# epitaque/RaytracingTest

Measured on AMD Instinct MI355X. Metric: Mrays/sec + achieved HBM GB/s, 1920x1080 primary rays, depth-10 SVO, higher is better.
Workload: dtype f32; 1 GPU; C3 depth-10 (1024^3) Custom1 SVO, 1920x1080 primary rays, flyover camera; svo_config=defaults, svo_nodes=1569748, svo_format=V2, stack_mode=hlsl, rays_per_gpu_step=2073600, parallelism=single

## Files before the change

raytracingtest_amd/csrc/svo_kernel.hip:

```cpp
#include "svo_traverse.h"
#include "svo_reflect.h"

#include <hipcub/hipcub.hpp>

namespace svo {
namespace {

__device__ __forceinline__ void mul4(const float *m, float v0, float v1, float v2, float v3, float out[3]) {
#pragma unroll
    for (int r = 0; r < 3; ++r) {
        float a = m[0 * 4 + r] * v0;
        a = a + m[1 * 4 + r] * v1;
        a = a + m[2 * 4 + r] * v2;
        a = a + m[3 * 4 + r] * v3;
        out[r] = a;
    }
}

__device__ __forceinline__ void normalize3(float v[3]) {
    float d = v[0] * v[0];
    d = d + v[1] * v[1];
    d = d + v[2] * v[2];
    float inv = 1.0f / sqrtf(d);
    v[0] = v[0] * inv;
// ... 684 lines not shown
        if (fin != 0) {
            if (SEGS && LM_ON(fin)) n_lane = (uint32_t)it;
            stopped |= stop;
            act &= ~fin;
            if (KG > 1) {
                recs |= fin & ~stop;
                act &= ~after_in_group<KG>(recs);
            }
        }
        asm volatile("s_cmp_lt_u32 %1, %2\n\ts_cselect_b64 %0, %3, 0" : "=s"(go) : "s"(it), "n"(MAX_ITERS), "s"(act) : "scc");
    } while (go != 0);
    if (LM_ON(act)) {
        r.flags |= 2u;
        if (SEGS) n_lane = (uint32_t)it;
    }
    stopped_lane = LM_ON(stopped);
    r.idx = sh ^ oct;
    r.trips = it;
}


__device__ __forceinline__ float beam_start(const LaunchParams &p, const FRay &f, int x, int gy) {
    if (!p.tile_start) return -__builtin_inff();
    const unsigned long long k = min(min(p.tile_start[(gy >> 3) * p.ts_tiles_x + (x >> 3)],
                                         p.tile_start[p.ts_super_off + (gy >> 6) * p.ts_super_x + (x >> 6)]),
                                     p.tile_start[p.ts_global_off]);
    const float d = (uint32_t)(k >> 32) == ~p.ts_gen ? __uint_as_float((uint32_t)k) : __builtin_inff();
    const float m = (2.0f * (fabsf(f.cx) + fabsf(f.cy) + fabsf(f.cz)) + fabsf(f.bx) + fabsf(f.by) + fabsf(f.bz)) *
                    0x1p-20f;
    const float s = d * (1.0f - 0x1p-16f) - m;
    return s == s ? s : -__builtin_inff();
}

template <int MODE, bool FA, bool COUNT = false, bool LOD = false>
__device__ __forceinline__ void trace_beam(const LaunchParams &p, FRay &f, uint2 *__restrict__ stk, float start) {
    uint32_t n_lane, armed_at;
    bool stopped;
    trace_seg<MODE, FA, false, COUNT, 0, LOD>(p, f, stk, start, __builtin_inff(), f.t_min >= start, n_lane, armed_at, stopped);
}

__device__ __forceinline__ int strip_col(int x, int m) {
    constexpr int K = STRIP_K;
    return K == 1 ? m * 8 + x : (m / K) * (8 * K) + x * K + (m % K);
}
__device__ __forceinline__ int strip_tile(int x, int e, int tiles_x, int tiles_y) {
    const int m = e / tiles_y, row = e - m * tiles_y;
    return row * tiles_x + strip_col(x, m);
}

template <int MODE, bool COUNT, bool FA, bool SH, bool LAT, bool LOD>
__device__ __forceinline__ void render_tile_body(const LaunchParams &p, int tiles_x) {
    static_assert(!(LOD && (SH || LAT)), "no LOD form of the fused shadow pass or the latency loop");
    extern __shared__ uint2 stk_base[];
    const int lane = threadIdx.x;
    const uint32_t t_entry = !COUNT && p.wave_log ? (uint32_t)__builtin_amdgcn_s_memrealtime() : 0u;
    const int n_tiles = (int)gridDim.x;
    const int t = p.tile_order ? (int)p.tile_order[blockIdx.x]
                : p.xcd_remap == 2 ? strip_tile((int)blockIdx.x % 8, (int)blockIdx.x / 8, tiles_x, n_tiles / tiles_x)
                                   : (int)blockIdx.x;
    const int bx = t % tiles_x, by = t / tiles_x;
    const int x = bx * 8 + (lane & 7);
    const int lr = by * 8 + (lane >> 3);
    if (x >= p.width || lr >= p.local_rows) return;
    if (p.tile_order && p.prio) {
        const uint32_t n = gridDim.x;
        const bool strips = p.xcd_remap == 2;
        const uint32_t b = strips ? blockIdx.x / 8 : blockIdx.x;
        const uint32_t *bound = strips ? p.tile_order + n + 4 + 4 * (blockIdx.x % 8) : p.tile_order + n;
        if (b < bound[0]) __builtin_amdgcn_s_setprio(3);
        else if (b < bound[1]) __builtin_amdgcn_s_setprio(2);
        else if (b < bound[2]) __builtin_amdgcn_s_setprio(1);
    }
    const int gy = global_row(p, lr);
    Ray r;
    {
        float org[3], dir[3];
        camera_ray(p.cam, p.width, p.height, x, gy, org, dir);
        setup_ray(org, dir, r);
    }
    uint2 *stk = stk_base + lane;
    uint32_t t0 = 0;
    if (!COUNT && p.wave_log) t0 = (uint32_t)__builtin_amdgcn_s_memrealtime();
    FRay f;
    to_fray(r, f);
    LeanDiag dg;
    if (LOD) {
        if (COUNT) {
            if (p.tile_start) trace_beam<MODE, false, true, true>(p, f, stk, fminf(beam_start(p, f, x, gy), p.lod_floor));
            else trace_lean<MODE, true, false, false, true, true>(p, f, stk);
        }
        else if (p.guard) trace_lean<MODE, true, false, false, false, true>(p, f, stk);
        else if (p.tile_start) trace_beam<MODE, FA, false, true>(p, f, stk, fminf(beam_start(p, f, x, gy), p.lod_floor));
        else trace_lean<MODE, false, false, FA, false, true>(p, f, stk);
    }
    else if (COUNT) {
        if (p.tile_start) trace_beam<MODE, false, true>(p, f, stk, beam_start(p, f, x, gy));
        else trace_lean<MODE, true, false, false, true>(p, f, stk);
    }
    else if (LAT) trace_lat<MODE>(p, f, stk);
    else if (!SH && p.wave_log) {
        if (p.guard) trace_lean<MODE, true, true>(p, f, stk, &dg);
        else trace_lean<MODE, false, true>(p, f, stk, &dg);
    }
    else if (p.guard) trace_lean<MODE, true>(p, f, stk);
    else if (p.tile_start) trace_beam<MODE, FA>(p, f, stk, beam_start(p, f, x, gy));
    else trace_lean<MODE, false, false, FA>(p, f, stk);
    from_fray(f, r);
    if (COUNT) {
        p.out.fetches[(size_t)lr * (size_t)p.width + (size_t)x] = r.fetches;
        return;
    }
    const float4 acc = accum_load(p, out_index(p, lr, gy, x));
    Record o;
    record(p, r, x, gy, o);
    int trips = f.trips;
    if (SH) {
        const bool hit = r.scale < S_MAX;
        const uint64_t hits = __ballot(hit);
        if (hits) {
            if (hit) {
                float so[3], sd[3];
                shadow_ray(p, x, gy, o.w[2], o.w[3], o.w[4], o.w[5], so, sd);
                Ray rs;
                setup_ray(so, sd, rs);
                FRay fs;
                to_fray(rs, fs);
                if (p.guard) trace_lean<MODE, true>(p, fs, stk);
                else trace_lean<MODE, false, false, FA>(p, fs, stk);
                from_fray(fs, rs);
                if (rs.scale < S_MAX) {
                    o.w[1] |= 8u << 16;
                    o.rgb[0] = o.rgb[1] = o.rgb[2] = 0.0f;
                }
                trips += fs.trips;
            }
            trips = __shfl(trips, __ffsll((long long)hits) - 1);
        }
    }
    if (p.out.hitmask) {
        const uint64_t hm = __ballot(r.scale < S_MAX);
        if (lane == 0) p.out.hitmask[t] = hm;
    }
    if (p.tile_cost && (!SH || lane == 0)) p.tile_cost[t] = (uint16_t)min(trips, 65535);
    if (p.wave_log && lane == 0) {
        uint32_t *w = p.wave_log + WAVE_LOG_WORDS * (size_t)blockIdx.x;
        w[8] = t_entry;
        w[10] = (uint32_t)__builtin_amdgcn_s_getreg((31 << 11) | 4);
        w[0] = t0;
        w[1] = (uint32_t)__builtin_amdgcn_s_memrealtime();
        w[2] = (uint32_t)t;
        w[3] = ((uint32_t)__builtin_amdgcn_s_getreg((31 << 11) | 20) & 0xFFu) | ((uint32_t)f.trips << 8);
        w[4] = (uint32_t)dg.loop_cycles;
        w[5] = (uint32_t)dg.fetch_cycles;
        w[6] = dg.fetch_trips;
        w[7] = dg.pop_trips;
    }
    store_outputs(p.out, out_index(p, lr, gy, x), o, acc);
    if (p.wave_log && lane == 0) p.wave_log[WAVE_LOG_WORDS * (size_t)blockIdx.x + 9] = (uint32_t)__builtin_amdgcn_s_memrealtime();
}

template <int MODE, bool COUNT, bool FA = false, bool SH = false, bool LAT = false>
#ifndef SVO_NUM_SGPR
#define SVO_NUM_SGPR 72
#endif
__global__ __launch_bounds__(TILE) __attribute__((amdgpu_num_sgpr(SVO_NUM_SGPR))) void render_tile_kernel(LaunchParams p, int tiles_x) {
    render_tile_body<MODE, COUNT, FA, SH, LAT, false>(p, tiles_x);
}

template <int MODE, bool COUNT, bool FA = false>
__global__ __launch_bounds__(TILE) __attribute__((amdgpu_num_sgpr(SVO_NUM_SGPR), amdgpu_waves_per_eu(8, 8)))
void render_tile_lod_kernel(LaunchParams p, int tiles_x) {
    render_tile_body<MODE, COUNT, FA, false, false, true>(p, tiles_x);
}

__device__ __forceinline__ int group_min(int v, int K) {
    v = min(v, __shfl_xor(v, 1));
    v = min(v, __shfl_xor(v, 2));
    if (K == 8) v = min(v, __shfl_xor(v, 4));
    return v;
}
__device__ __forceinline__ float group_get(float v, int K, int j) {
    return __shfl(v, (int)(threadIdx.x & ~(uint32_t)(K - 1)) + j);
}
__device__ __forceinline__ uint32_t group_get(uint32_t v, int K, int j) {
    return (uint32_t)__shfl((int)v, (int)(threadIdx.x & ~(uint32_t)(K - 1)) + j);
}

__device__ __forceinline__ void seg_rebalance(uint2 *slot, float t_entry, float t_start, float t_end, uint32_t c,
                                              int f, int K, float tot, float *hint8, bool store) {
    const int lane = (int)threadIdx.x, k = lane & (K - 1);
    slot[lane] = make_uint2(k <= f ? c : 0u, __float_as_uint(k == 0 ? t_entry : k > f ? t_end : t_start));
    __syncthreads();
    if (k != 0 || !store) return;
    if (!(tot > 0.0f)) {
        hint8[0] = __int_as_float(0x7FC00000);
        return;
    }
    const uint2 *g = slot + lane;
    int m = 0;
    float cum = 0.0f, cm = (float)g[0].x, t0 = t_entry, prev = 0.0f;
    float t1 = K > 1 ? __uint_as_float(g[1].y) : t_end;
// ... 80 lines not shown
    tot += (uint32_t)__shfl_xor((int)tot, 2);
    if (K == 8) tot += (uint32_t)__shfl_xor((int)tot, 4);
    seg_rebalance(stk_base, t_entry, t_start, t_end, c, fsel, K, (float)tot, hint8, inside && hint8);
    if (p.tile_cost) {
        uint32_t m = inside ? tot : 0u;
        for (int d = K; d < TILE; d <<= 1) m = max(m, (uint32_t)__shfl_xor((int)m, d));
        if (lane == 0) {
            p.part_cost[SEG_KMAX * (size_t)t + part] = (uint16_t)min(m, (uint32_t)(SEG_COST_FLAG - 1));
            if (part == 0) p.tile_cost[t] = (uint16_t)(SEG_COST_FLAG | K);
        }
    }
    if (p.out.hitmask) {
        uint32_t hit_w = (writer && inside && r.scale < S_MAX) ? 1u : 0u;
        hit_w |= (uint32_t)__shfl_xor((int)hit_w, 1);
        hit_w |= (uint32_t)__shfl_xor((int)hit_w, 2);
        if (K == 8) hit_w |= (uint32_t)__shfl_xor((int)hit_w, 4);
        const uint64_t hm = __ballot(k == 0 && hit_w != 0);
        uint32_t bits = 0;
#pragma unroll
        for (int j = 0; j < R; ++j) bits |= (uint32_t)((hm >> (K * j)) & 1ull) << j;
        if (lane == 0) {
            if (K == 4) reinterpret_cast<uint16_t *>(p.out.hitmask)[4 * (size_t)t + part] = (uint16_t)bits;
            else reinterpret_cast<uint8_t *>(p.out.hitmask)[8 * (size_t)t + part] = (uint8_t)bits;
        }
    }
    if (LOG) seg_log(p, 9, now_100mhz());
    if (!writer || !inside) return;
    const float4 acc = accum_load(p, out_index(p, lr, gy, x));
    Record o;
    record(p, r, x, gy, o);
    store_outputs(p.out, out_index(p, lr, gy, x), o, acc);
}

template <int MODE, bool FA, bool LAT, bool LOG>
#ifndef SVO_SEG_WAVES_PER_EU
#define SVO_SEG_WAVES_PER_EU 8
#endif
__global__ __launch_bounds__(TILE) __attribute__((amdgpu_num_sgpr(SVO_NUM_SGPR), amdgpu_waves_per_eu(SVO_SEG_WAVES_PER_EU, 8)))
void render_seg_kernel(LaunchParams p, int tiles_x) {
    extern __shared__ uint2 stk_base[];
    const int lane = threadIdx.x;
    const uint32_t t_in = LOG ? now_100mhz() : 0u;
    const uint32_t entry = p.tile_order[blockIdx.x];
    if (LOG) {
        seg_log(p, 8, t_in);
        seg_log(p, 2, entry);
    }
    if (entry == SEG_EMPTY) return;
    const int t = (int)(entry & 0x0FFFFFFFu);
    const int code = (int)(entry >> 28);
    if (p.prio) {
        const uint32_t *bound = p.tile_order + gridDim.x + 4 + 4 * (blockIdx.x % 8);
        const uint32_t b = blockIdx.x / 8;
        if (b < bound[0]) __builtin_amdgcn_s_setprio(3);
        else if (b < bound[1]) __builtin_amdgcn_s_setprio(2);
        else if (b < bound[2]) __builtin_amdgcn_s_setprio(1);
    }
    const int bx = t % tiles_x, by = t / tiles_x;
    uint2 *stk = stk_base + lane;
    if (code == 0) {
        const int x = bx * 8 + (lane & 7);
        const int lr = by * 8 + (lane >> 3);
        if (x >= p.width || lr >= p.local_rows) return;
        const int gy = global_row(p, lr);
        Ray r;
        {
            float org[3], dir[3];
            camera_ray(p.cam, p.width, p.height, x, gy, org, dir);
            setup_ray(org, dir, r);
        }
        FRay f;
        to_fray(r, f);
        if (LOG) seg_log(p, 0, now_100mhz());
        if (LAT) trace_lat<MODE>(p, f, stk);
        else if (p.tile_start) trace_beam<MODE, FA>(p, f, stk, beam_start(p, f, x, gy));
        else trace_lean<MODE, false, false, FA>(p, f, stk);
        if (LOG) {
            seg_log(p, 1, now_100mhz());
            seg_log(p, 3, ((uint32_t)__builtin_amdgcn_s_getreg((31 << 11) | 20) & 0xFFu) | ((uint32_t)f.trips << 8));
        }
        from_fray(f, r);
        const float4 acc = accum_load(p, out_index(p, lr, gy, x));
        Record o;
        record(p, r, x, gy, o);
        if (p.out.hitmask) {
            const uint64_t hm = __ballot(r.scale < S_MAX);
            if (lane == 0) p.out.hitmask[t] = hm;
        }
        if (p.tile_cost) p.tile_cost[t] = (uint16_t)min(f.trips, (int)(SEG_COST_FLAG - 1));
        store_outputs(p.out, out_index(p, lr, gy, x), o, acc);
        if (LOG) seg_log(p, 9, now_100mhz());
        return;
    }
    if (code <= 4) seg_part<MODE, FA, 4, LOG>(p, stk_base, t, code - 1, bx, by);
    else seg_part<MODE, FA, 8, LOG>(p, stk_base, t, code - 5, bx, by);
}

template <int MODE, bool FA, bool LOD>
__device__ __forceinline__ void render_samples_body(const LaunchParams &p, int tiles_x) {
    extern __shared__ uint2 stk_base[];
    const int lane = threadIdx.x & (TILE - 1);
    const int k = threadIdx.x / TILE;
    const int n_tiles = (int)gridDim.x;
    const int t = p.tile_order ? (int)p.tile_order[blockIdx.x]
                : p.xcd_remap == 2 ? strip_tile((int)blockIdx.x % 8, (int)blockIdx.x / 8, tiles_x, n_tiles / tiles_x)
                                   : (int)blockIdx.x;
    const int bx = t % tiles_x, by = t / tiles_x;
// ... 541 lines not shown
                rgb[0] = rgb[1] = rgb[2] = 0.0f;
            } else {
                float alb[3];
                decode_dxt(at.x, at.y, (int)(c.y & 0xFFu), alb);
                shade_hit(a.cam, n, alb, rgb);
            }
        }
    } else if (a.out.rgba || a.out.rgba8) {
        float org[3], dir[3];
        camera_ray(a.cam, a.width, a.height, x, y, org, dir);
        sky(dir[1], rgb);
    }
    if (a.out.hits) {
        uint2 *d = reinterpret_cast<uint2 *>(a.out.hits + dst);
        d[0] = make_uint2(c.x, c.y);
        d[1] = make_uint2(c.z, __float_as_uint(n[0]));
        d[2] = make_uint2(__float_as_uint(n[1]), __float_as_uint(n[2]));
    }
    if (a.out.rgba) a.out.rgba[dst] = make_float4(rgb[0], rgb[1], rgb[2], 1.0f);
    if (a.out.rgba8) a.out.rgba8[dst] = pack_rgba8(rgb[0], rgb[1], rgb[2]);
}

}

static size_t lds_pad() {
    static const size_t pad = [] {
        const char *v = std::getenv("SVO_LDS_PAD");
        return v ? (size_t)std::strtoul(v, nullptr, 10) : (size_t)0;
    }();
    return pad;
}

template <int MODE, bool COUNT>
static hipError_t launch_variant(const LaunchParams &p, hipStream_t stream) {
    const int bx = (p.width + 7) / 8, by = (p.local_rows + 7) / 8;
    const size_t lds = (size_t)p.slots * TILE * sizeof(uint2) + lds_pad();
    const dim3 grid((unsigned)(bx * by)), block(TILE);
    if (p.lod) {
        if (p.seg > 0 || p.lat || p.shadows) return hipErrorInvalidValue;
        const bool fa = p.fetch_all && !p.guard;
        if (COUNT)
            hipLaunchKernelGGL((render_tile_lod_kernel<MODE, true>), grid, block, lds, stream, p, bx);
        else if (p.samples > 0) {
            const size_t per = (size_t)std::max(p.slots, 2) * TILE * sizeof(uint2);
            const dim3 sblock((unsigned)(TILE * p.samples));
            if (fa) hipLaunchKernelGGL((render_samples_lod_kernel<MODE, true>), grid, sblock, per * p.samples, stream, p, bx);
            else hipLaunchKernelGGL((render_samples_lod_kernel<MODE, false>), grid, sblock, per * p.samples, stream, p, bx);
        } else if (fa)
            hipLaunchKernelGGL((render_tile_lod_kernel<MODE, false, true>), grid, block, lds, stream, p, bx);
        else
            hipLaunchKernelGGL((render_tile_lod_kernel<MODE, false, false>), grid, block, lds, stream, p, bx);
        return hipGetLastError();
    }
    if (!COUNT && p.samples > 0) {
        const size_t per = (size_t)std::max(p.slots, 2) * TILE * sizeof(uint2);
        const dim3 sblock((unsigned)(TILE * p.samples));
        if (p.fetch_all && !p.guard)
            hipLaunchKernelGGL((render_samples_kernel<MODE, true>), grid, sblock, per * p.samples, stream, p, bx);
        else
            hipLaunchKernelGGL((render_samples_kernel<MODE, false>), grid, sblock, per * p.samples, stream, p, bx);
        return hipGetLastError();
    }
    if (!COUNT && p.seg > 0) {
        const dim3 sgrid((unsigned)order_strips_grid(bx * by, p.seg, p.seg_kmax));
        if (p.lat && p.wave_log)
            hipLaunchKernelGGL((render_seg_kernel<MODE, true, true, true>), sgrid, block, 2 * lds, stream, p, bx);
        else if (p.lat)
            hipLaunchKernelGGL((render_seg_kernel<MODE, true, true, false>), sgrid, block, 2 * lds, stream, p, bx);
        else if (p.fetch_all && p.wave_log)
            hipLaunchKernelGGL((render_seg_kernel<MODE, true, false, true>), sgrid, block, lds, stream, p, bx);
        else if (p.fetch_all)
            hipLaunchKernelGGL((render_seg_kernel<MODE, true, false, false>), sgrid, block, lds, stream, p, bx);
        else if (p.wave_log)
            hipLaunchKernelGGL((render_seg_kernel<MODE, false, false, true>), sgrid, block, lds, stream, p, bx);
        else
            hipLaunchKernelGGL((render_seg_kernel<MODE, false, false, false>), sgrid, block, lds, stream, p, bx);
        return hipGetLastError();
    }
    if (COUNT)
        hipLaunchKernelGGL((render_tile_kernel<MODE, true>), grid, block, lds, stream, p, bx);
    else if (p.lat)
        hipLaunchKernelGGL((render_tile_kernel<MODE, false, false, false, true>), grid, block, 2 * lds, stream, p, bx);
    else if (p.shadows == 2) {
        if (p.fetch_all && !p.guard)
            hipLaunchKernelGGL((render_tile_kernel<MODE, false, true, true>), grid, block, lds, stream, p, bx);
        else
            hipLaunchKernelGGL((render_tile_kernel<MODE, false, false, true>), grid, block, lds, stream, p, bx);
    } else if (p.fetch_all && !p.guard)
        hipLaunchKernelGGL((render_tile_kernel<MODE, false, true>), grid, block, lds, stream, p, bx);
    else
        hipLaunchKernelGGL((render_tile_kernel<MODE, false>), grid, block, lds, stream, p, bx);
    return hipGetLastError();
}

template <int MODE>
static hipError_t launch_query_mode(const LaunchParams &p, const QueryArgs &q, hipStream_t stream) {
    const size_t lds = (size_t)p.slots * TILE * sizeof(uint2) + lds_pad();
    const dim3 grid((q.n + (uint32_t)TILE - 1u) / (uint32_t)TILE), block(TILE);
    if (p.lod) {
        if (p.guard)
            hipLaunchKernelGGL((query_rays_lod_kernel<MODE, true, false>), grid, block, lds, stream, p, q);
        else if (p.fetch_all)
            hipLaunchKernelGGL((query_rays_lod_kernel<MODE, false, true>), grid, block, lds, stream, p, q);
        else
            hipLaunchKernelGGL((query_rays_lod_kernel<MODE, false, false>), grid, block, lds, stream, p, q);
        return hipGetLastError();
    }
    if (p.guard)
        hipLaunchKernelGGL((query_rays_kernel<MODE, true, false>), grid, block, lds, stream, p, q);
    else if (p.fetch_all)
        hipLaunchKernelGGL((query_rays_kernel<MODE, false, true>), grid, block, lds, stream, p, q);
    else
// ... 714 lines not shown
hipError_t launch_beam_splat(const BeamParams &b, hipStream_t stream) {
    if (b.n_boxes == 0) return hipSuccess;
    const uint32_t per_wg = SPLAT_THREADS * SPLAT_PER;
    hipLaunchKernelGGL(beam_splat_kernel, dim3((b.n_boxes + per_wg - 1u) / per_wg), dim3(SPLAT_THREADS), 0, stream, b);
    return hipGetLastError();
}

template <int MODE>
static hipError_t launch_shadows(const LaunchParams &p, hipStream_t stream) {
    const int bx = (p.width + 7) / 8, by = (p.local_rows + 7) / 8;
    const size_t lds = (size_t)p.slots * TILE * sizeof(uint2);
    if (p.fetch_all && !p.guard)
        hipLaunchKernelGGL((shadow_tile_kernel<MODE, true>), dim3((unsigned)(bx * by)), dim3(TILE), lds, stream, p, bx);
    else
        hipLaunchKernelGGL((shadow_tile_kernel<MODE>), dim3((unsigned)(bx * by)), dim3(TILE), lds, stream, p, bx);
    return hipGetLastError();
}

__global__ __launch_bounds__(256) void beam_starts_kernel(LaunchParams p) {
    const size_t i = (size_t)blockIdx.x * blockDim.x + threadIdx.x;
    if (i >= (size_t)p.width * (size_t)p.local_rows) return;
    const int x = (int)(i % (size_t)p.width), lr = (int)(i / (size_t)p.width);
    const int gy = global_row(p, lr);
    Ray r;
    float org[3], dir[3];
    camera_ray(p.cam, p.width, p.height, x, gy, org, dir);
    setup_ray(org, dir, r);
    FRay f;
    to_fray(r, f);
    p.out.starts[i] = beam_start(p, f, x, gy);
}

hipError_t launch_render(const LaunchParams &p, int stack_mode, hipStream_t stream, hipEvent_t primary_start,
                         hipEvent_t primary_end) {
    if (p.out.starts) {
        const size_t n = (size_t)p.width * (size_t)p.local_rows;
        hipLaunchKernelGGL(beam_starts_kernel, dim3((unsigned)((n + 255) / 256)), dim3(256), 0, stream, p);
        return hipGetLastError();
    }
    const bool count = p.out.fetches != nullptr;
    hipError_t e = hipSuccess;
    if (primary_start && (e = hipEventRecord(primary_start, stream)) != hipSuccess) return e;
    if (stack_mode == 0)
        e = count ? launch_variant<0, true>(p, stream) : launch_variant<0, false>(p, stream);
    else
        e = count ? launch_variant<1, true>(p, stream) : launch_variant<1, false>(p, stream);
    if (e != hipSuccess) return e;
    if (primary_end && (e = hipEventRecord(primary_end, stream)) != hipSuccess) return e;
    if (!count && p.shadows == 1 && (p.out.hits || p.out.compact))
        return stack_mode == 0 ? launch_shadows<0>(p, stream) : launch_shadows<1>(p, stream);
    if (!count && p.shadows == 3 && (p.out.hits || p.out.compact) && p.out.hitmask) {
        if ((e = launch_pack<true>(nullptr, p.width, p.local_rows, p.out.hitmask, stream)) != hipSuccess) return e;
        const int n = ((p.width + 7) / 8) * ((p.local_rows + 7) / 8);
        const SparseLayout L = sparse_layout(n, p.width * p.local_rows, 4);
        const uint8_t *base = reinterpret_cast<const uint8_t *>(p.out.hitmask);
        const uint32_t *list = reinterpret_cast<const uint32_t *>(base + L.rgb);
        const uint32_t *cnt = reinterpret_cast<const uint32_t *>(base + L.offsets) + n;
        const size_t lds = (size_t)p.slots * TILE * sizeof(uint2);
        const dim3 grid((unsigned)(((size_t)p.width * (size_t)p.local_rows + TILE - 1) / TILE));
        LaunchParams q = p;
        q.out.hitmask = nullptr;
        if (stack_mode == 0) {
            if (p.fetch_all && !p.guard) hipLaunchKernelGGL((shadow_list_kernel<0, true>), grid, dim3(TILE), lds, stream, q, list, cnt);
            else hipLaunchKernelGGL((shadow_list_kernel<0>), grid, dim3(TILE), lds, stream, q, list, cnt);
        } else {
            if (p.fetch_all && !p.guard) hipLaunchKernelGGL((shadow_list_kernel<1, true>), grid, dim3(TILE), lds, stream, q, list, cnt);
            else hipLaunchKernelGGL((shadow_list_kernel<1>), grid, dim3(TILE), lds, stream, q, list, cnt);
        }
        return hipGetLastError();
    }
    return hipSuccess;
}

template <int MODE>
static hipError_t launch_reflect_mode(const LaunchParams &q, const uint32_t *list, const uint32_t *cnt, const ReflectArgs &ra,
                                      hipStream_t stream) {
    const size_t lds = (size_t)q.slots * TILE * sizeof(uint2);
    const dim3 grid((unsigned)(((size_t)q.width * (size_t)q.local_rows + TILE - 1) / TILE)), block(TILE);
    const float sr = ra.specular[0], sg = ra.specular[1], sb = ra.specular[2];
// ... 52 lines not shown
```

raytracingtest_amd/csrc/svo_rt.hip:

```cpp
#include <hip/hip_runtime.h>

#include <algorithm>
#include <cmath>
#include <atomic>
#include <condition_variable>
#include <cstdint>
#include <cstdio>
#include <cstdlib>
#include <cstring>
#include <deque>
#include <memory>
#include <mutex>
#include <string>
#include <thread>
#include <vector>

#include "svo_rt.h"
#include "svo_beam.h"
#include "svo_lod.h"
#include "svo_sched.h"
#include "svo_traverse.h"

namespace {

// ... 686 lines not shown
    o.compact = reinterpret_cast<uint32_t *>(f->compact);
    o.position = reinterpret_cast<float4 *>(f->position);
    o.voxel = reinterpret_cast<unsigned long long *>(f->voxel);
    o.rgb8 = f->rgb8;
    o.hitmask = reinterpret_cast<unsigned long long *>(f->hitmask);
    o.frame_layout = f->layout == SVO_LAYOUT_FRAME ? 1 : 0;
    return o;
}

struct SampleArgs {
    int n;
    const float *offsets;
    uint32_t first;
    float4 *accum;
    uint32_t *rgba8;
    uint8_t *rgb8;
    int layout;
};

struct LaunchPlan {
    Deal b;
    int stack_mode = 0;
    hipStream_t s = nullptr;
    Sched *q = nullptr;
    Geo key;
    Geo okey;
    int seg_cap = 0, n_tiles = 0;
    int mode_now = 0;
    int used_kpack = 0;
    bool instr = false;
    bool jittered = false;
    bool latency_bound = false;
    bool beam_planned = false;
    size_t n_wave = 0;
};

void base_params(const svo_ctx *ctx, const LaunchPlan &L, int width, int height, const svo::Outputs &out,
                 svo::LaunchParams &p) {
    const Deal &b = L.b;
    const int stack_mode = L.stack_mode;
    std::memset(&p, 0, sizeof p);
    p.nodes = ctx->d_nodes;
    p.att = ctx->d_att;
    p.n_nodes = (uint32_t)std::min<size_t>(ctx->n_nodes, 0xFFFFFFFFu);
    p.cam = ctx->cam;
    p.width = width;
    p.height = height;
    p.band_rows = b.rows;
    p.band_rank = b.rank;
    p.band_count = b.count;
    p.band_cycle = b.cycle;
    for (int i = 0; i < b.cycle; ++i)
        if (b.owner[i] == b.rank) p.band_pos[p.band_cnt++] = (uint8_t)i;
    p.local_rows = band_rows_local(height, b);
    p.slots = std::max(ctx->depth - 1, 1);
    p.guard = !ctx->depth_exact || (stack_mode == 0 && ctx->n_nodes > ((size_t)1 << 24)) ||
              ctx->n_nodes >= ((size_t)1 << 29);
    p.fetch_all = ctx->fetch_all >= 0 ? ctx->fetch_all : (ctx->n_nodes < ((size_t)1 << 24) ? 1 : 0);
    p.out = out;
    if (b.count == 1) p.out.frame_layout = 0;
    p.xcd_remap = ctx->xcd_remap;
    if (p.xcd_remap == 2 && ((width + 7) / 8) % (8 * svo::STRIP_K) != 0) p.xcd_remap = 0;
    p.shadows = (ctx->options & SVO_OPT_SHADOW_RAYS) ? (ctx->shadow_compact ? 3 : ctx->fused_shadows ? 2 : 1) : 0;
}

int sample_forms(svo_ctx *ctx, LaunchPlan &L, svo::LaunchParams &p, const SampleArgs *sa) {
// ... 354 lines not shown
                gen = 0;
            }
            if (!reuse) ++gen;
            bp.boxes = db.d;
            bp.n_boxes = db.n;
            bp.tile_start = buf;
            bp.gen = gen;
            bp.diag = ctx->beam_diag;
            bp.tiles_x = tx;
            bp.tiles_y = ty;
            bp.super_x = sx;
            bp.super_y = sy;
            bp.super_off = tx * ty;
            bp.global_off = tx * ty + sx * sy;
            bp.width = width;
            bp.height = height;
            if (!reuse) {
                hipError_t eb = svo::launch_beam_splat(bp, s);
                if (eb != hipSuccess) return fail(SVO_ERR_HIP, std::string("beam splat launch: ") + hipGetErrorString(eb));
                if (q) {
                    q->held_splat = li == 1;
                    q->ts_view = ctx->view_gen;
                    q->ts_boxes = bid;
                    q->ts_w = width;
                    q->ts_h = height;
                }
            }
            p.tile_start = buf;
            p.ts_gen = gen;
            p.ts_tiles_x = tx;
            p.ts_super_x = sx;
            p.ts_super_off = bp.super_off;
            p.ts_global_off = bp.global_off;
        }
    }
    return SVO_OK;
}

int render_and_reorder(svo_ctx *ctx, LaunchPlan &L, svo::LaunchParams &p) {
    Sched *q = L.q;
    const hipStream_t s = L.s;
    const Geo &key = L.key, &okey = L.okey;
    const int mode_now = L.mode_now;
    hipEvent_t ev0 = nullptr, ev1 = nullptr;
    if (!L.instr) {
        int rc = take_events(ctx, STAGE_KERNEL, &ev0, &ev1);
        if (rc) return rc;
    }
    hipError_t e = svo::launch_render(p, L.stack_mode, s, ev0, ev1);
    if (e != hipSuccess) return fail(SVO_ERR_HIP, std::string("render launch: ") + hipGetErrorString(e));
    bool refresh = false;
    bool moving_build = false;
    if (q && p.tile_cost) {
        const unsigned long long n = q->launches++;
        const bool moving = q->view_prev != ctx->view_gen;
        q->view_prev = ctx->view_gen;
        q->off_prev[0] = p.cam.px_off[0];
        q->off_prev[1] = p.cam.px_off[1];
        const bool drift = q->built_cost != ctx->cost_gen || p.samples != 0 || L.jittered;
        const bool relayout = svo_sched::other_layout(ctx->relayout != 0, p.tile_order != nullptr, p.seg, p.seg_kmax, L.used_kpack,
                                                      okey.seg, svo::seg_kmax_of(okey.kpack), okey.kpack);
        if (relayout) q->relayout_pending = true;
        const bool own_layout = !relayout && q->relayout_pending;
        refresh = svo_sched::needs_refresh(q->order_key != okey, n, ctx->order_every, drift, q->built_mode != mode_now, own_layout,
                                           q->held_splat, q->built_view != ctx->view_gen, moving, n - q->last_build,
                                           ctx->move_every);
        q->held_splat = false;
        if (own_layout) q->relayout_pending = false;
        if (refresh) q->last_build = n;
        moving_build = moving;
    }
    if (refresh) {
        const int r = q->stats_head;
        uint32_t *st16 = q->stats ? q->stats + 16 * r : nullptr;
        const int bi = q->next_buf;
        q->next_buf ^= 1;
        HIP_TRY(hipEventRecord(q->render_done, s));
        HIP_TRY(hipStreamWaitEvent(q->side, q->render_done, 0));
        e = p.xcd_remap == 2 ? svo::launch_order_strips(p.tile_cost, q->order_buf[bi], L.n_tiles, (p.width + 7) / 8, q->side,
                                                        st16, okey.seg, p.part_cost, okey.kpack,
                                                        moving_build && ctx->spread ? 1 : 0)
                             : svo::launch_order_tiles(p.tile_cost, q->order_buf[bi], L.n_tiles, q->side, st16);
// ... 431 lines not shown
    k.beam = c->beam;
    k.beam_back = c->beam_back;
    k.beam_back_held = c->beam_back_held;
    k.shadow_form = c->shadow_compact ? 2 : c->fused_shadows ? 0 : 1;
    k.shadow_order = c->shadow_order_enabled;
    k.readback = c->pin_push;
    k.host_copy_threads = c->host_copy_threads;
    k.sparse_payload = c->sparse_payload;
    k.peer_copy = c->peer_copy;
    *o = k;
}

int check_config(const svo_config &k) {
    auto bit = [](int32_t v) { return v == 0 || v == 1; };
    auto table = [](uint32_t t) {
        if (t > 0xFFFFFFu) return false;
        for (int c = 0; c < 6; ++c) {
            const uint32_t kc = (t >> (4 * c)) & 15u;
            if (kc != 0 && kc != 4 && kc != 8) return false;
        }
        return true;
    };
    auto ratio = [](float r) { return std::isfinite(r) && r >= 0.0f; };
    const char *bad = !bit(k.tile_order) ? "tile_order" : !bit(k.xcd_strips) ? "xcd_strips"
                    : !bit(k.issue_priority) ? "issue_priority" : k.order_every < 1 ? "order_every"
                    : k.move_every < 1 ? "move_every" : !bit(k.move_spread) ? "move_spread"
                    : !bit(k.relayout) ? "relayout" : k.fetch_all < -1 || k.fetch_all > 1 ? "fetch_all"
                    : k.loop_form < -1 || k.loop_form > 1 ? "loop_form" : !ratio(k.lat_ratio) ? "lat_ratio"
                    : !bit(k.segments) ? "segments" : !table(k.seg_table_latency) ? "seg_table_latency"
                    : !table(k.seg_table_issue) ? "seg_table_issue" : !table(k.seg_table_thin) ? "seg_table_thin"
                    : !ratio(k.seg_ratio) ? "seg_ratio" : !ratio(k.seg_thin_ratio) ? "seg_thin_ratio"
                    : k.seg_cap < 1 ? "seg_cap" : k.seg_min_chain < 0 ? "seg_min_chain"
                    : k.seg_move < 1 || k.seg_move > 2 ? "seg_move" : k.seg_jitter < 0 || k.seg_jitter > 2 ? "seg_jitter"
                    : k.seg_all != 0 && k.seg_all != 4 && k.seg_all != 8 ? "seg_all" : !bit(k.beam) ? "beam"
                    : k.beam_back < 0 || k.beam_back > 22 ? "beam_back" : k.shadow_form < 0 || k.shadow_form > 2 ? "shadow_form"
                    : !bit(k.shadow_order) ? "shadow_order" : k.readback < 0 || k.readback > 2 ? "readback"
                    : k.host_copy_threads < 0 || k.host_copy_threads > 16 ? "host_copy_threads"
                    : !bit(k.sparse_payload) ? "sparse_payload" : !bit(k.peer_copy) ? "peer_copy"
                    : k.beam_back_held < -1 || k.beam_back_held > 22 ? "beam_back_held" : nullptr;
    if (bad) return fail(SVO_ERR_ARG, std::string("svo_config.") + bad + " out of range");
    return SVO_OK;
}

int apply_config(svo_ctx *c, const svo_config &k) {
    c->tile_order = k.tile_order;
    c->xcd_remap = k.xcd_strips ? 2 : 0;
    c->prio = k.issue_priority;
    c->order_every = k.order_every;
    c->move_every = k.move_every;
    c->spread = k.move_spread;
    c->relayout = k.relayout;
    c->fetch_all = k.fetch_all;
    c->lat_mode = k.loop_form;
    c->lat_ratio = k.lat_ratio;
    c->seg_mode = k.segments;
    c->seg_kpack_lat = (int)k.seg_table_latency;
    c->seg_kpack_issue = (int)k.seg_table_issue;
    c->seg_kpack_thin = (int)k.seg_table_thin;
    c->seg_ratio = k.seg_ratio;
    c->thin_ratio = k.seg_thin_ratio;
    c->seg_cap = k.seg_cap;
    c->seg_min_chain = k.seg_min_chain;
    c->seg_move = k.seg_move;
    c->seg_jitter = k.seg_jitter;
    c->seg_all = k.seg_all;
    c->seg_scramble = k.seg_scramble;
    c->shadow_compact = k.shadow_form == 2;
    c->fused_shadows = k.shadow_form == 0;
    c->shadow_order_enabled = k.shadow_order;
    c->sparse_payload = k.sparse_payload;
    c->peer_copy = k.peer_copy;
    if (c->pin_push != k.readback) {
        if (c->h_pin[0]) {
            HIP_TRY(hipSetDevice(c->device));
            HIP_TRY(hipStreamSynchronize(c->stream));
            if (c->copy_stream) HIP_TRY(hipStreamSynchronize(c->copy_stream));
            if (c->copy_stream2) HIP_TRY(hipStreamSynchronize(c->copy_stream2));
            free_pinned(c);
        }
        c->pin_push = k.readback;
    }
    if (c->host_copy_threads != k.host_copy_threads) {
        c->copy_pool.reset();
        c->host_copy_threads = k.host_copy_threads;
    }
    const bool boxes = c->beam != k.beam || c->beam_back != k.beam_back || c->beam_back_held != k.beam_back_held;
    c->beam = k.beam;
    c->beam_back = k.beam_back;
    c->beam_back_held = k.beam_back_held;
    if (boxes && c->n_nodes > 0) {
        const int rc = recompute_pool(c);
        if (rc) return rc;
    }
    for (Sched &q : c->sched) {
        q.lat_key = Geo();
        q.lat_mode = -1;
    }
    return SVO_OK;
}

int order_query_scratch(svo_ctx *c, hipStream_t s) {
    if (c->q_valid && c->q_stream != s) {
        if (!c->q_event) HIP_TRY(hipEventCreateWithFlags(&c->q_event, hipEventDisableTiming));
        HIP_TRY(hipEventRecord(c->q_event, c->q_stream));
        HIP_TRY(hipStreamWaitEvent(s, c->q_event, 0));
    }
    c->q_stream = s;
    c->q_valid = true;
    return SVO_OK;
}

template <class T>
int grow_query_scratch(T **buf, size_t *cap, size_t need) {
    if (need <= *cap) return SVO_OK;
    HIP_TRY(hipDeviceSynchronize());
    return regrow(buf, cap, need, need);
}

constexpr size_t MAX_QUERY_RAYS = ((size_t)1 << 31) - 1;
// ... 1103 lines not shown
```

raytracingtest_amd/csrc/svo_traverse.h:

```cpp
#pragma once
#include <hip/hip_runtime.h>
#include <stdint.h>

#include <algorithm>

#include "svo_sky.h"

namespace svo {

constexpr int S_MAX = 23;
constexpr int MAX_ITERS = 65536;
constexpr int TILE = 64;
constexpr int MAX_PARTS = 64;
constexpr int WAVE_LOG_WORDS = 12;
constexpr int MAX_CYCLE = 256;
constexpr int MAX_SAMPLES = 8;
#ifdef SVO_STRIP_K
constexpr int STRIP_K = SVO_STRIP_K;
#else
constexpr int STRIP_K = 1;
#endif

struct Camera {
    float c2w[16];
// ... 103 lines not shown
inline size_t order_strips_entries(int n_tiles, int seg_cap, int kmax = SEG_KMAX) {
    return (size_t)order_strips_grid(n_tiles, seg_cap, kmax) + 36;
}

struct BeamParams {
    const uint2 *boxes;
    uint32_t n_boxes;
    unsigned long long *tile_start;
    uint32_t gen;
    uint32_t diag;
    int tiles_x, tiles_y, super_x, super_y, super_off, global_off;
    int width, height;
    float org[3];
    float minv[9];
    float plane[4][3];
};
hipError_t launch_beam_splat(const BeamParams &b, hipStream_t stream);

hipError_t launch_accumulate(float4 *dst, const float4 *src, size_t n_px, uint32_t sample, int num_cus,
                             hipStream_t stream);

hipError_t launch_assemble(const AssembleParams &a, hipStream_t stream);

hipError_t launch_pack_hits(const uint8_t *rgb8, int width, int local_rows, void *part, hipStream_t stream);
size_t shadow_list_bytes(int width, int local_rows);

hipError_t launch_push_host(const void *src, void *dst_mapped, size_t bytes, int blocks, hipStream_t stream);

hipError_t launch_pack_rgb8(const float4 *src, uint8_t *dst, size_t n_px, int num_cus, hipStream_t stream);

hipError_t launch_pack_rgba8(const float4 *src, uint32_t *dst, size_t n_px, int num_cus, hipStream_t stream);

hipError_t launch_render(const LaunchParams &p, int stack_mode, hipStream_t stream, hipEvent_t primary_start = nullptr,
                         hipEvent_t primary_end = nullptr);

struct ReflectArgs {
    void *scratch;
    float specular[3];
    int max_bounces;
    svo_sky::Texture sky;
};
hipError_t launch_reflect(const LaunchParams &p, const ReflectArgs &ra, int stack_mode, hipStream_t stream);

hipError_t launch_sky_fill(const LaunchParams &p, const svo_sky::Texture &sky, const unsigned long long *masks,
                           hipStream_t stream);
hipError_t launch_sample_sky(const svo_sky::Texture &sky, const float4 *dirs, uint32_t n, float4 *out,
                             hipStream_t stream);

struct QueryRay {
    float org[3];
    float t_max;
    float dir[3];
    uint32_t reserved;
};
static_assert(sizeof(QueryRay) == 32, "ray record layout");
constexpr uint32_t QUERY_RAW = 2u;
constexpr uint32_t HIT_INVALID_RAY = 0x10u;
constexpr uint32_t QUERY_KEY_BITS = 30;
struct QueryArgs {
    const QueryRay *rays;
    uint32_t n;
    uint32_t flags;
    const uint32_t *index;
    Outputs out;
};
hipError_t launch_query(const LaunchParams &p, const QueryArgs &q, int stack_mode, hipStream_t stream);
hipError_t launch_query_keys(const QueryArgs &q, uint32_t *keys, uint32_t *index, hipStream_t stream);
// ... 8 lines not shown
```

Baseline: 27060 Mrays/s.

## Add beam miss fast path that writes sky for fully-missing tiles

Adds a new beam mode (beam==2) where each wave reads its beam-splat bound. When every lane has no hit bound and a sane ray, the wave skips traversal and writes sky/miss records directly. Other waves reuse the already-read bound instead of recomputing it. This only runs when beam is set to 2, so with default settings it likely does not run. It adds kernel variants and risks differences in the outputs if the miss test is wrong.

```diff
diff --git a/raytracingtest_amd/csrc/svo_kernel.hip b/raytracingtest_amd/csrc/svo_kernel.hip
--- a/raytracingtest_amd/csrc/svo_kernel.hip
+++ b/raytracingtest_amd/csrc/svo_kernel.hip
@@ -740,6 +740,42 @@
     return s == s ? s : -__builtin_inff();
 }
 
+__device__ __forceinline__ float beam_bound(const LaunchParams &p, int x, int gy) {
+    const unsigned long long k = min(min(p.tile_start[(gy >> 3) * p.ts_tiles_x + (x >> 3)],
+                                         p.tile_start[p.ts_super_off + (gy >> 6) * p.ts_super_x + (x >> 6)]),
+                                     p.tile_start[p.ts_global_off]);
+    return (uint32_t)(k >> 32) == ~p.ts_gen ? __uint_as_float((uint32_t)k) : __builtin_inff();
+}
+__device__ __forceinline__ float beam_start_at(const FRay &f, float d) {
+    const float m = (2.0f * (fabsf(f.cx) + fabsf(f.cy) + fabsf(f.cz)) + fabsf(f.bx) + fabsf(f.by) + fabsf(f.bz)) *
+                    0x1p-20f;
+    const float s = d * (1.0f - 0x1p-16f) - m;
+    return s == s ? s : -__builtin_inff();
+}
+
+__device__ __forceinline__ bool beam_all_miss(float d, const float org[3], const float dir[3]) {
+    const float lo = 0x1p-100f, far = 0x1p20f;
+    const bool lane = d == __builtin_inff() && fabsf(dir[0]) >= lo && fabsf(dir[1]) >= lo && fabsf(dir[2]) >= lo &&
+                      fabsf(to_svo(org[0])) < far && fabsf(to_svo(org[1])) < far && fabsf(to_svo(org[2])) < far;
+    return __all(lane) != 0;
+}
+
+__device__ __forceinline__ void miss_tile(const LaunchParams &p, int t, int x, int lr, int gy, float dir_y) {
+    const size_t i = out_index(p, lr, gy, x);
+    const float4 acc = accum_load(p, i);
+    Record o;
+    o.w[0] = 0xFFFFFFFFu; o.w[1] = 0u; o.w[2] = 0x7F800000u;
+    o.w[3] = 0u; o.w[4] = 0u; o.w[5] = 0u;
+    sky(dir_y, o.rgb);
+    o.pos[0] = o.pos[1] = o.pos[2] = 0.0f;
+    o.key = ~0ull;
+    if (threadIdx.x == 0) {
+        if (p.out.hitmask) p.out.hitmask[t] = 0ull;
+        if (p.tile_cost) p.tile_cost[t] = (uint16_t)1;
+    }
+    store_outputs(p.out, i, o, acc);
+}
+
 template <int MODE, bool FA, bool COUNT = false, bool LOD = false>
 __device__ __forceinline__ void trace_beam(const LaunchParams &p, FRay &f, uint2 *__restrict__ stk, float start) {
     uint32_t n_lane, armed_at;
@@ -756,9 +792,10 @@
     return row * tiles_x + strip_col(x, m);
 }
 
-template <int MODE, bool COUNT, bool FA, bool SH, bool LAT, bool LOD>
+template <int MODE, bool COUNT, bool FA, bool SH, bool LAT, bool LOD, bool MISS = false>
 __device__ __forceinline__ void render_tile_body(const LaunchParams &p, int tiles_x) {
     static_assert(!(LOD && (SH || LAT)), "no LOD form of the fused shadow pass or the latency loop");
+    static_assert(!(MISS && (LOD || LAT)), "no miss path in the LOD kernels or the latency loop");
     extern __shared__ uint2 stk_base[];
     const int lane = threadIdx.x;
     const uint32_t t_entry = !COUNT && p.wave_log ? (uint32_t)__builtin_amdgcn_s_memrealtime() : 0u;
@@ -781,9 +818,18 @@
     }
     const int gy = global_row(p, lr);
     Ray r;
+    float bd = __builtin_inff();
     {
         float org[3], dir[3];
         camera_ray(p.cam, p.width, p.height, x, gy, org, dir);
+        if (MISS && p.tile_start) {
+            bd = beam_bound(p, x, gy);
+            if ((COUNT || (!p.wave_log && !p.guard)) && beam_all_miss(bd, org, dir)) {
+                if (COUNT) p.out.fetches[(size_t)lr * (size_t)p.width + (size_t)x] = 0u;
+                else miss_tile(p, t, x, lr, gy, dir[1]);
+                return;
+            }
+        }
         setup_ray(org, dir, r);
     }
     uint2 *stk = stk_base + lane;
@@ -802,7 +848,8 @@
         else trace_lean<MODE, false, false, FA, false, true>(p, f, stk);
     }
     else if (COUNT) {
-        if (p.tile_start) trace_beam<MODE, false, true>(p, f, stk, beam_start(p, f, x, gy));
+        if (MISS && p.tile_start) trace_beam<MODE, false, true>(p, f, stk, beam_start_at(f, bd));
+        else if (p.tile_start) trace_beam<MODE, false, true>(p, f, stk, beam_start(p, f, x, gy));
         else trace_lean<MODE, true, false, false, true>(p, f, stk);
     }
     else if (LAT) trace_lat<MODE>(p, f, stk);
@@ -811,6 +858,7 @@
         else trace_lean<MODE, false, true>(p, f, stk, &dg);
     }
     else if (p.guard) trace_lean<MODE, true>(p, f, stk);
+    else if (MISS && p.tile_start) trace_beam<MODE, FA>(p, f, stk, beam_start_at(f, bd));
     else if (p.tile_start) trace_beam<MODE, FA>(p, f, stk, beam_start(p, f, x, gy));
     else trace_lean<MODE, false, false, FA>(p, f, stk);
     from_fray(f, r);
@@ -875,6 +923,12 @@
     render_tile_body<MODE, COUNT, FA, SH, LAT, false>(p, tiles_x);
 }
 
+template <int MODE, bool COUNT, bool FA = false, bool SH = false>
+__global__ __launch_bounds__(TILE) __attribute__((amdgpu_num_sgpr(SVO_NUM_SGPR)))
+void render_tile_kernel_miss(LaunchParams p, int tiles_x) {
+    render_tile_body<MODE, COUNT, FA, SH, false, false, true>(p, tiles_x);
+}
+
 template <int MODE, bool COUNT, bool FA = false>
 __global__ __launch_bounds__(TILE) __attribute__((amdgpu_num_sgpr(SVO_NUM_SGPR), amdgpu_waves_per_eu(8, 8)))
 void render_tile_lod_kernel(LaunchParams p, int tiles_x) {
@@ -1021,12 +1075,13 @@
     store_outputs(p.out, out_index(p, lr, gy, x), o, acc);
 }
 
-template <int MODE, bool FA, bool LAT, bool LOG>
 #ifndef SVO_SEG_WAVES_PER_EU
 #define SVO_SEG_WAVES_PER_EU 8
 #endif
+template <int MODE, bool FA, bool LAT, bool LOG, bool MISS = false>
 __global__ __launch_bounds__(TILE) __attribute__((amdgpu_num_sgpr(SVO_NUM_SGPR), amdgpu_waves_per_eu(SVO_SEG_WAVES_PER_EU, 8)))
 void render_seg_kernel(LaunchParams p, int tiles_x) {
+    static_assert(!(MISS && (LAT || LOG)), "no miss path in the latency form or the logged kernels");
     extern __shared__ uint2 stk_base[];
     const int lane = threadIdx.x;
     const uint32_t t_in = LOG ? now_100mhz() : 0u;
@@ -1053,15 +1108,24 @@
         if (x >= p.width || lr >= p.local_rows) return;
         const int gy = global_row(p, lr);
         Ray r;
+        float bd = __builtin_inff();
         {
             float org[3], dir[3];
             camera_ray(p.cam, p.width, p.height, x, gy, org, dir);
+            if (MISS && p.tile_start) {
+                bd = beam_bound(p, x, gy);
+                if (beam_all_miss(bd, org, dir)) {
+                    miss_tile(p, t, x, lr, gy, dir[1]);
+                    return;
+                }
+            }
             setup_ray(org, dir, r);
         }
         FRay f;
         to_fray(r, f);
         if (LOG) seg_log(p, 0, now_100mhz());
         if (LAT) trace_lat<MODE>(p, f, stk);
+        else if (MISS && p.tile_start) trace_beam<MODE, FA>(p, f, stk, beam_start_at(f, bd));
         else if (p.tile_start) trace_beam<MODE, FA>(p, f, stk, beam_start(p, f, x, gy));
         else trace_lean<MODE, false, false, FA>(p, f, stk);
         if (LOG) {
@@ -1669,7 +1733,7 @@
 }
 
 template <int MODE, bool COUNT>
-static hipError_t launch_variant(const LaunchParams &p, hipStream_t stream) {
+static hipError_t launch_variant(const LaunchParams &p, hipStream_t stream, bool miss) {
     const int bx = (p.width + 7) / 8, by = (p.local_rows + 7) / 8;
     const size_t lds = (size_t)p.slots * TILE * sizeof(uint2) + lds_pad();
     const dim3 grid((unsigned)(bx * by)), block(TILE);
@@ -1700,7 +1764,10 @@
     }
     if (!COUNT && p.seg > 0) {
         const dim3 sgrid((unsigned)order_strips_grid(bx * by, p.seg, p.seg_kmax));
-        if (p.lat && p.wave_log)
+        if (miss && p.tile_start && !p.lat && !p.wave_log) {
+            if (p.fetch_all) hipLaunchKernelGGL((render_seg_kernel<MODE, true, false, false, true>), sgrid, block, lds, stream, p, bx);
+            else hipLaunchKernelGGL((render_seg_kernel<MODE, false, false, false, true>), sgrid, block, lds, stream, p, bx);
+        } else if (p.lat && p.wave_log)
             hipLaunchKernelGGL((render_seg_kernel<MODE, true, true, true>), sgrid, block, 2 * lds, stream, p, bx);
         else if (p.lat)
             hipLaunchKernelGGL((render_seg_kernel<MODE, true, true, false>), sgrid, block, 2 * lds, stream, p, bx);
@@ -1714,7 +1781,17 @@
             hipLaunchKernelGGL((render_seg_kernel<MODE, false, false, false>), sgrid, block, lds, stream, p, bx);
         return hipGetLastError();
     }
-    if (COUNT)
+    if (miss && p.tile_start && (COUNT || (!p.lat && !p.wave_log && !p.guard))) {
+        if (COUNT)
+            hipLaunchKernelGGL((render_tile_kernel_miss<MODE, true>), grid, block, lds, stream, p, bx);
+        else if (p.shadows == 2) {
+            if (p.fetch_all) hipLaunchKernelGGL((render_tile_kernel_miss<MODE, false, true, true>), grid, block, lds, stream, p, bx);
+            else hipLaunchKernelGGL((render_tile_kernel_miss<MODE, false, false, true>), grid, block, lds, stream, p, bx);
+        } else if (p.fetch_all)
+            hipLaunchKernelGGL((render_tile_kernel_miss<MODE, false, true>), grid, block, lds, stream, p, bx);
+        else
+            hipLaunchKernelGGL((render_tile_kernel_miss<MODE, false>), grid, block, lds, stream, p, bx);
+    } else if (COUNT)
         hipLaunchKernelGGL((render_tile_kernel<MODE, true>), grid, block, lds, stream, p, bx);
     else if (p.lat)
         hipLaunchKernelGGL((render_tile_kernel<MODE, false, false, false, true>), grid, block, 2 * lds, stream, p, bx);
@@ -2495,7 +2572,7 @@
 }
 
 hipError_t launch_render(const LaunchParams &p, int stack_mode, hipStream_t stream, hipEvent_t primary_start,
-                         hipEvent_t primary_end) {
+                         hipEvent_t primary_end, bool miss) {
     if (p.out.starts) {
         const size_t n = (size_t)p.width * (size_t)p.local_rows;
         hipLaunchKernelGGL(beam_starts_kernel, dim3((unsigned)((n + 255) / 256)), dim3(256), 0, stream, p);
@@ -2505,9 +2582,9 @@
     hipError_t e = hipSuccess;
     if (primary_start && (e = hipEventRecord(primary_start, stream)) != hipSuccess) return e;
     if (stack_mode == 0)
-        e = count ? launch_variant<0, true>(p, stream) : launch_variant<0, false>(p, stream);
+        e = count ? launch_variant<0, true>(p, stream, miss) : launch_variant<0, false>(p, stream, miss);
     else
-        e = count ? launch_variant<1, true>(p, stream) : launch_variant<1, false>(p, stream);
+        e = count ? launch_variant<1, true>(p, stream, miss) : launch_variant<1, false>(p, stream, miss);
     if (e != hipSuccess) return e;
     if (primary_end && (e = hipEventRecord(primary_end, stream)) != hipSuccess) return e;
     if (!count && p.shadows == 1 && (p.out.hits || p.out.compact))
diff --git a/raytracingtest_amd/csrc/svo_rt.hip b/raytracingtest_amd/csrc/svo_rt.hip
--- a/raytracingtest_amd/csrc/svo_rt.hip
+++ b/raytracingtest_amd/csrc/svo_rt.hip
@@ -742,6 +742,7 @@
     bool jittered = false;
     bool latency_bound = false;
     bool beam_planned = false;
+    bool beam_miss = false;
     size_t n_wave = 0;
 };
 
@@ -1162,6 +1163,7 @@
             p.ts_super_x = sx;
             p.ts_super_off = bp.super_off;
             p.ts_global_off = bp.global_off;
+            L.beam_miss = ctx->beam == 2;
         }
     }
     return SVO_OK;
@@ -1177,7 +1179,7 @@
         int rc = take_events(ctx, STAGE_KERNEL, &ev0, &ev1);
         if (rc) return rc;
     }
-    hipError_t e = svo::launch_render(p, L.stack_mode, s, ev0, ev1);
+    hipError_t e = svo::launch_render(p, L.stack_mode, s, ev0, ev1, L.beam_miss);
     if (e != hipSuccess) return fail(SVO_ERR_HIP, std::string("render launch: ") + hipGetErrorString(e));
     bool refresh = false;
     bool moving_build = false;
@@ -1675,7 +1677,7 @@
                     : !ratio(k.seg_ratio) ? "seg_ratio" : !ratio(k.seg_thin_ratio) ? "seg_thin_ratio"
                     : k.seg_cap < 1 ? "seg_cap" : k.seg_min_chain < 0 ? "seg_min_chain"
                     : k.seg_move < 1 || k.seg_move > 2 ? "seg_move" : k.seg_jitter < 0 || k.seg_jitter > 2 ? "seg_jitter"
-                    : k.seg_all != 0 && k.seg_all != 4 && k.seg_all != 8 ? "seg_all" : !bit(k.beam) ? "beam"
+                    : k.seg_all != 0 && k.seg_all != 4 && k.seg_all != 8 ? "seg_all" : k.beam < 0 || k.beam > 2 ? "beam"
                     : k.beam_back < 0 || k.beam_back > 22 ? "beam_back" : k.shadow_form < 0 || k.shadow_form > 2 ? "shadow_form"
                     : !bit(k.shadow_order) ? "shadow_order" : k.readback < 0 || k.readback > 2 ? "readback"
                     : k.host_copy_threads < 0 || k.host_copy_threads > 16 ? "host_copy_threads"
@@ -1727,7 +1729,7 @@
         c->copy_pool.reset();
         c->host_copy_threads = k.host_copy_threads;
     }
-    const bool boxes = c->beam != k.beam || c->beam_back != k.beam_back || c->beam_back_held != k.beam_back_held;
+    const bool boxes = !c->beam != !k.beam || c->beam_back != k.beam_back || c->beam_back_held != k.beam_back_held;
     c->beam = k.beam;
     c->beam_back = k.beam_back;
     c->beam_back_held = k.beam_back_held;
diff --git a/raytracingtest_amd/csrc/svo_traverse.h b/raytracingtest_amd/csrc/svo_traverse.h
--- a/raytracingtest_amd/csrc/svo_traverse.h
+++ b/raytracingtest_amd/csrc/svo_traverse.h
@@ -159,7 +159,7 @@
 hipError_t launch_pack_rgba8(const float4 *src, uint32_t *dst, size_t n_px, int num_cus, hipStream_t stream);
 
 hipError_t launch_render(const LaunchParams &p, int stack_mode, hipStream_t stream, hipEvent_t primary_start = nullptr,
-                         hipEvent_t primary_end = nullptr);
+                         hipEvent_t primary_end = nullptr, bool miss = false);
 
 struct ReflectArgs {
     void *scratch;
```

Result: slower. 26750 Mrays/s (-1.1%).
